# sentiric/sentiric-stt-whisper-service

Hardware: NVIDIA B200
Metric: audio-sec/sec (RTFx) (higher is better)
Workload: dtype bf16 (f32 accumulate)

## Files before the change

include/sw_whisper.h:

```cpp
#ifndef SW_WHISPER_H
#define SW_WHISPER_H

#include <stddef.h>
#include <stdint.h>

#ifdef __cplusplus
extern "C" {
#endif

#define SW_API __attribute__((visibility("default")))

typedef struct sw_ctx sw_ctx;
typedef struct sw_result sw_result;

SW_API const char* sw_last_error(void);
SW_API const char* sw_version(void);
SW_API int sw_device_count(void);

typedef void (*sw_log_callback)(int level, const char* text, void* user);
SW_API void sw_log_set(sw_log_callback cb, void* user);

typedef struct sw_ctx_params {
  int device;
  int max_batch;
// ... 56 lines not shown
                         int n_samples, sw_result** out);
SW_API int sw_full_batch_pcm16(sw_ctx* ctx, const sw_full_params* params,
                               const int16_t* const* pcm16, const int* n_samples, int n,
                               sw_result** out);
SW_API int sw_full_batch_f32(sw_ctx* ctx, const sw_full_params* params, const float* const* pcm,
                             const int* n_samples, int n, sw_result** out);
SW_API int sw_full_batch_pcm16_lang(sw_ctx* ctx, const sw_full_params* params, const int16_t* const* pcm16,
                                    const int* n_samples, int n, const char* const* languages, sw_result** out);
SW_API int sw_full_batch_f32_lang(sw_ctx* ctx, const sw_full_params* params, const float* const* pcm,
                                  const int* n_samples, int n, const char* const* languages, sw_result** out);
SW_API void* sw_host_alloc(size_t bytes);
SW_API void sw_host_free(void* p);

typedef struct sw_token_data {
  int32_t id, tid;
  float p, plog, pt, ptsum;
  int64_t t0, t1, t_dtw;
  float vlen;
} sw_token_data;
SW_API int sw_result_n_segments(const sw_result* r);
SW_API const char* sw_result_segment_text(const sw_result* r, int i);
SW_API int64_t sw_result_segment_t0(const sw_result* r, int i);
SW_API int64_t sw_result_segment_t1(const sw_result* r, int i);
SW_API int sw_result_segment_speaker_turn_next(const sw_result* r, int i);
SW_API int sw_result_n_tokens(const sw_result* r, int i);
SW_API sw_token_data sw_result_token_data(const sw_result* r, int i, int j);
SW_API int sw_result_lang_id(const sw_result* r);
SW_API int sw_result_n_decode_steps(const sw_result* r);
SW_API int sw_result_n_windows(const sw_result* r);
SW_API void sw_result_free(sw_result* r);

typedef struct sw_stats {
  double ms_mel, ms_encode, ms_decode;
  long n_windows, n_steps, n_launches;
  double decode_bytes;
  double decoder_weight_bytes;
  double h2d_bytes, d2h_bytes;
  double ms_xattn;
  long n_xattn;
  double xattn_bytes;
  long n_lanes;
} sw_stats;
SW_API void sw_ctx_set_kernel_timing(sw_ctx* ctx, int on);
SW_API int sw_ctx_get_stats(sw_ctx* ctx, sw_stats* out, int reset);

typedef struct sw_prosody_opts {
  float lpf_alpha, gender_threshold, min_pitch, max_pitch;
} sw_prosody_opts;
enum { SW_EMOTION_NEUTRAL = 0, SW_EMOTION_EXCITED = 1, SW_EMOTION_SAD = 2, SW_EMOTION_ANGRY = 3 };
typedef struct sw_prosody {
  char gender;
  int emotion;
  float arousal, valence, pitch_mean, pitch_std, energy_mean, energy_std, spectral_centroid,
      zero_crossing_rate;
  float speaker_vec[8];
} sw_prosody;
SW_API sw_prosody_opts sw_prosody_default_opts(void);
SW_API int sw_prosody_segments_f32(sw_ctx* ctx, const float* pcm, int64_t n_samples, int sample_rate,
                                   const int64_t* seg_begin, const int64_t* seg_end, int n_segs,
                                   const sw_prosody_opts* opts, sw_prosody* out);
SW_API int sw_prosody_segments_pcm16(sw_ctx* ctx, const int16_t* pcm, int64_t n_samples, int sample_rate,
                                     const int64_t* seg_begin, const int64_t* seg_end, int n_segs,
                                     const sw_prosody_opts* opts, sw_prosody* out);

SW_API int64_t sw_resample_out_len(int64_t n_in, int sr_in, int sr_out);
SW_API int sw_resample_f32(sw_ctx* ctx, const float* in, int64_t n_in, int sr_in, int sr_out, float* out);

SW_API int sw_mel_pcm16(sw_ctx* ctx, const int16_t* pcm, int n_samples, float* out, int* n_len);
SW_API int sw_mel_f32(sw_ctx* ctx, const float* pcm, int n_samples, float* out, int* n_len);
SW_API int sw_encode(sw_ctx* ctx, const float* mel, int n_windows, float* out);
SW_API int sw_decode_logits(sw_ctx* ctx, const int32_t* tokens, int n_windows, int n_tok,
                            float* logits);

SW_API int sw_dev_gemm_bf16(const void* dA, const void* dB, void* dC, const float* d_bias,
                            const float* d_residual, int M, int N, int K, int lda, int ldb, int ldc,
                            int flags, int block_n, void* stream);

SW_API int sw_dev_skinny_gemm(const void* dX, const void* dW, int R, int N, int K, const float* d_bias,
                              int gelu, void* d_out, float* d_partial, int split, void* stream);
SW_API int sw_dev_skinny_split(int N, int K);
SW_API int sw_dev_skinny_gemm_k(int kernel, const void* dX, const void* dW, int R, int N, int K, const float* d_bias,
                                int gelu, void* d_out, float* d_partial, int split, void* stream);
SW_API int sw_dev_skinny_split_k(int kernel, int N, int K);
SW_API int sw_dev_layer_norm(float* d_x, int rows, int d, const float* g, const float* b,
                             void* d_out_bf16, const float* d_partial, int n_split, const float* d_bias,
                             void* stream);
SW_API int sw_dev_occupy(int n_ctas, int smem_bytes, float ms, size_t stream_bytes);

#ifdef __cplusplus
}
#endif
#endif
```

sentiric-stt-whisper-service_b200/csrc/attn_enc_tc.cu:

```cuda
#include <stdlib.h>

#include "common.cuh"
#include "gemm.cuh"
#include "kernels.cuh"

namespace sw {
namespace {

constexpr int TQ = 128, TK = 128, DH = 64;
constexpr int TILE_BYTES = 128 * 64 * 2;
constexpr int SM_Q = 0, SM_K = TILE_BYTES, SM_V = 3 * TILE_BYTES;
constexpr int SM_BARS = 5 * TILE_BYTES;
constexpr int SM_XCH = SM_BARS + 128;
constexpr int ATT_SMEM = SM_XCH + 512;
constexpr int ATT_THREADS = 320;
constexpr int TMEM_COLS = 256, TM_P = 128, TM_O = 192;
#ifndef SW_ATT_POLY
#define SW_ATT_POLY 0
#endif
constexpr bool ATT_POLY = SW_ATT_POLY != 0;

__device__ __forceinline__ uint64_t make_umma_desc_mn_sw128(uint32_t smem_addr) {
  uint64_t d = 0;
  d |= static_cast<uint64_t>((smem_addr >> 4) & 0x3FFF);
  d |= static_cast<uint64_t>(1) << 16;
  d |= static_cast<uint64_t>(64) << 32;
  d |= static_cast<uint64_t>(1) << 46;
  d |= static_cast<uint64_t>(2) << 61;
  return d;
}

__device__ __forceinline__ float fast_exp2(float x) {
  float y;
  asm("ex2.approx.ftz.f32 %0, %1;" : "=f"(y) : "f"(x));
  return y;
}

__device__ __forceinline__ float exp2_fma(float x) {
  x = fmaxf(x, -125.f);
  const float t = x + 12582912.f;
  const float f = x - (t - 12582912.f);
  float p = fmaf(f, 0.05550411f, 0.24022651f);
  p = fmaf(p, f, 0.69314718f);
  p = fmaf(p, f, 1.0f);
  return __int_as_float(__float_as_int(p) + (__float_as_int(t) << 23));
}

template <bool LAGGED>
__global__ void __launch_bounds__(ATT_THREADS, 2)
encoder_attention_tc_kernel(const __grid_constant__ CUtensorMap map_qkv, bf16* __restrict__ out, int T, int d,
                            long long* __restrict__ trace) {
  extern __shared__ __align__(1024) uint8_t smem[];
  uint64_t* bars = reinterpret_cast<uint64_t*>(smem + SM_BARS);
  uint64_t* q_full = bars;
  uint64_t* k_full = bars + 1;
  uint64_t* v_full = bars + 3;
  uint64_t* kv_empty = bars + 5;
  uint64_t* s_full = bars + 7;
  uint64_t* p_ready = bars + 8;
  uint64_t* o_full = bars + 9;
  uint64_t* o_free = bars + 10;
  uint32_t* tmem_slot = reinterpret_cast<uint32_t*>(bars + 11);

  const int qt = blockIdx.x, h = blockIdx.y, w = blockIdx.z;
  const int warp = __shfl_sync(0xffffffffu, threadIdx.x >> 5, 0), lane = threadIdx.x & 31;
  const int q0 = qt * TQ;
  const int n_tiles = (T + TK - 1) / TK;
  const bool tr = trace && blockIdx.x == 5 && blockIdx.y == 7 && blockIdx.z == (gridDim.z >> 1);
#define ATT_TRACE(role, tile, ev)                                                        \
  do {                                                                                   \
    if (tr) trace[((role) * 16 + (tile)) * 8 + (ev)] = clock64();                        \
  } while (0)
  const int row_base = w * T;

  if (threadIdx.x == 0) {
    if (smem_u32(smem) & 1023) {
      printf("encoder_attention_tc: shared memory base not 1024-byte aligned\n");
      __trap();
    }
    tma_prefetch_desc(&map_qkv);
    mbar_init(q_full, 1);
    for (int s = 0; s < 2; ++s) {
      mbar_init(&k_full[s], 1);
      mbar_init(&v_full[s], 1);
      mbar_init(&kv_empty[s], 1);
    }
    mbar_init(s_full, 1);
    mbar_init(p_ready, 8);
    mbar_init(o_full, 1);
    mbar_init(o_free, 8);
    fence_mbar_init();
  }
  if (warp == 1) {
    tmem_alloc(tmem_slot, TMEM_COLS);
    tmem_relinquish();
  }
  tc_fence_before();
  __syncthreads();
  tc_fence_after();
  const uint32_t tmem = *tmem_slot;

  if (warp == 0) {
    if (elect_one_sync()) {
      mbar_arrive_expect_tx(q_full, TILE_BYTES);
      tma_load_2d(smem + SM_Q, &map_qkv, q_full, h * DH, row_base + q0);
      for (int j = 0; j < n_tiles; ++j) {
        const int s = j & 1;
        const uint32_t ph = (j >> 1) & 1;
        mbar_wait(&kv_empty[s], ph ^ 1);
        mbar_arrive_expect_tx(&k_full[s], TILE_BYTES);
        tma_load_2d(smem + SM_K + s * TILE_BYTES, &map_qkv, &k_full[s], d + h * DH, row_base + j * TK);
        mbar_arrive_expect_tx(&v_full[s], TILE_BYTES);
        tma_load_2d(smem + SM_V + s * TILE_BYTES, &map_qkv, &v_full[s], 2 * d + h * DH, row_base + j * TK);
      }
    }
  } else if (warp == 1) {
    if (elect_one_sync()) {
      constexpr uint32_t idesc_s = make_idesc_bf16(128, 128);
      constexpr uint32_t idesc_o = make_idesc_bf16(128, 64) | (1u << 16);
      const uint32_t sq = smem_u32(smem + SM_Q);
      mbar_wait(q_full, 0);
      auto issue_s = [&](int j) {
        const int s = j & 1;
        mbar_wait(&k_full[s], (j >> 1) & 1);
        tc_fence_after();
        const uint64_t adesc = make_umma_desc_sw128(sq);
        const uint64_t bdesc = make_umma_desc_sw128(smem_u32(smem + SM_K + s * TILE_BYTES));
#pragma unroll
        for (int k = 0; k < DH / 16; ++k) umma_bf16(tmem, adesc + 2 * k, bdesc + 2 * k, idesc_s, k != 0);
        umma_commit(s_full);
      };
      issue_s(0);
      for (int j = 0; j < n_tiles; ++j) {
        const int s = j & 1;
        const uint32_t ph = (j >> 1) & 1;
        const uint32_t sv = smem_u32(smem + SM_V + s * TILE_BYTES);
        ATT_TRACE(1, j, 0);
        mbar_wait(p_ready, j & 1);
        tc_fence_after();
        ATT_TRACE(1, j, 1);
        if (j + 1 < n_tiles) issue_s(j + 1);
        ATT_TRACE(1, j, 2);
        mbar_wait(o_free, j & 1);
        tc_fence_after();
        mbar_wait(&v_full[s], ph);
        tc_fence_after();
#pragma unroll
        for (int k = 0; k < TK / 16; ++k) {
          const uint64_t bdesc = make_umma_desc_mn_sw128(sv + k * 2048);
          umma_bf16_ts(tmem + TM_O, tmem + TM_P + k * 8, bdesc, idesc_o, k != 0);
        }
        umma_commit(o_full);
        umma_commit(&kv_empty[s]);
        ATT_TRACE(1, j, 3);
      }
    }
  } else {
    const int qd = warp & 3;
    const int half = (warp - 2) >> 2;
    const int row = qd * 32 + lane;
    const uint32_t lane_addr = static_cast<uint32_t>(qd * 32) << 16;
    const float sc = 0.125f * 1.4426950408889634f;
    float m = -INFINITY, l = 0.f;
    float acc[DH / 2];
#pragma unroll
    for (int i = 0; i < DH / 2; ++i) acc[i] = 0.f;
    uint16_t* xch = reinterpret_cast<uint16_t*>(smem + SM_XCH);
    float alpha_prev = 1.f;
    auto fold_o = [&](int j, float a) {
      mbar_wait(o_full, j & 1);
      tc_fence_after();
      uint32_t r[32];
      tmem_ld_32x32b_x32(tmem + lane_addr + TM_O + half * 32, r);
      tmem_ld_wait(r);
#pragma unroll
      for (int i = 0; i < 32; ++i) acc[i] = acc[i] * a + __uint_as_float(r[i]);
      tc_fence_before();
    };
    const uint32_t s_addr = tmem + lane_addr + half * 64;
    const uint32_t p_addr = tmem + lane_addr + TM_P + half * 32;
    float shift_prev = 0.f;
    for (int j = 0; j < n_tiles; ++j) {
      const int valid = min(TK, T - j * TK);
      mbar_wait(s_full, j & 1);
      tc_fence_after();
      if (warp == 2 && lane == 0) ATT_TRACE(0, j, 0);
      auto exchange_max = [&](float mx) {
        const uint32_t u = __float_as_uint(mx);
        uint32_t t = u & 0xffff0000u;
        if (t != u && !(u >> 31)) t += 0x10000u;
        mx = __uint_as_float(t);
        xch[half * 128 + row] = static_cast<uint16_t>(t >> 16);
        asm volatile("bar.sync 1, 256;" ::: "memory");
        return fmaxf(mx, __uint_as_float(static_cast<uint32_t>(xch[(half ^ 1) * 128 + row]) << 16));
      };
      float lsum = 0.f, mx = -INFINITY;
      auto sweep = [&](float shift, bool want_p) {
        lsum = 0.f;
        mx = -INFINITY;
#pragma unroll
        for (int cc = 0; cc < 2; ++cc) {
          const int c = half * 2 + cc;
          uint32_t r[32];
          tmem_ld_32x32b_x32(s_addr + cc * 32, r);
          tmem_ld_wait(r);
          const bool full = c * 32 + 32 <= valid;
          if (full) {
#pragma unroll
            for (int i = 0; i < 32; ++i) mx = fmaxf(mx, __uint_as_float(r[i]));
          } else {
#pragma unroll
            for (int i = 0; i < 32; ++i)
              if (c * 32 + i < valid) mx = fmaxf(mx, __uint_as_float(r[i]));
          }
          if (!want_p) continue;
          uint32_t pk[16];
          if (full) {
#pragma unroll
            for (int i = 0; i < 16; ++i) {
              const float p0 = fast_exp2(__uint_as_float(r[2 * i]) * sc - shift);
              const float x1 = __uint_as_float(r[2 * i + 1]) * sc - shift;
              const float p1 = (ATT_POLY && i % 3 != 2) ? exp2_fma(x1) : fast_exp2(x1);
              lsum += p0 + p1;
              pk[i] = pack_bf16x2(p0, p1);
            }
          } else {
#pragma unroll
            for (int i = 0; i < 16; ++i) {
              float p0 = fast_exp2(__uint_as_float(r[2 * i]) * sc - shift);
              float p1 = fast_exp2(__uint_as_float(r[2 * i + 1]) * sc - shift);
              if (c * 32 + 2 * i >= valid) p0 = 0.f;
              if (c * 32 + 2 * i + 1 >= valid) p1 = 0.f;
              lsum += p0 + p1;
              pk[i] = pack_bf16x2(p0, p1);
            }
          }
          if (cc == 0 && j > 0) {
            mbar_wait(o_full, (j - 1) & 1);
            tc_fence_after();
          }
          tmem_st_32x32b_x16(p_addr + cc * 16, pk);
        }
      };
      float shift;
      if (!LAGGED || j == 0) {
        sweep(0.f, false);
        if (warp == 2 && lane == 0) ATT_TRACE(0, j, 1);
        mx = exchange_max(mx);
        if (warp == 2 && lane == 0) ATT_TRACE(0, j, 2);
        m = fmaxf(m, mx * sc);
        shift = m;
        sweep(shift, true);
      } else {
        shift = m;
        sweep(shift, true);
        if (warp == 2 && lane == 0) ATT_TRACE(0, j, 1);
        mx = exchange_max(mx);
        if (warp == 2 && lane == 0) ATT_TRACE(0, j, 2);
        m = fmaxf(m, mx * sc);
        if (__any_sync(0xffffffffu, m - shift > 60.f)) {
          shift = m;
          sweep(shift, true);
        }
      }
      const float alpha = j == 0 ? 1.f : fast_exp2(shift_prev - shift);
      shift_prev = shift;
      l = l * alpha + lsum;
      if (warp == 2 && lane == 0) ATT_TRACE(0, j, 3);
      tmem_st_wait();
      tc_fence_before();
      __syncwarp();
      if (lane == 0) mbar_arrive(p_ready);
      if (warp == 2 && lane == 0) ATT_TRACE(0, j, 4);
      if (j > 0) fold_o(j - 1, alpha_prev);
      __syncwarp();
      if (lane == 0) mbar_arrive(o_free);
      if (warp == 2 && lane == 0) ATT_TRACE(0, j, 5);
      alpha_prev = alpha;
    }
    fold_o(n_tiles - 1, alpha_prev);
    float* lx = reinterpret_cast<float*>(smem + SM_K);
    asm volatile("bar.sync 1, 256;" ::: "memory");
    lx[half * 128 + row] = l;
    asm volatile("bar.sync 1, 256;" ::: "memory");
    l += lx[(half ^ 1) * 128 + row];
    if (q0 + row < T) {
      const float inv = 1.0f / l;
      bf16* op = out + (int64_t)(row_base + q0 + row) * d + h * DH + half * 32;
#pragma unroll
      for (int i = 0; i < 4; ++i) {
        uint4 o;
        o.x = pack_bf16x2(acc[8 * i] * inv, acc[8 * i + 1] * inv);
        o.y = pack_bf16x2(acc[8 * i + 2] * inv, acc[8 * i + 3] * inv);
        o.z = pack_bf16x2(acc[8 * i + 4] * inv, acc[8 * i + 5] * inv);
        o.w = pack_bf16x2(acc[8 * i + 6] * inv, acc[8 * i + 7] * inv);
        reinterpret_cast<uint4*>(op)[i] = o;
      }
    }
  }

  tc_fence_before();
  __syncthreads();
  if (warp == 1) {
    tc_fence_after();
    tmem_dealloc(tmem, TMEM_COLS);
  }
}

}

int encoder_attention_tc(const bf16* qkv, bf16* out, int n_win, int T, int d, int n_head, cudaStream_t stream) {
  if (n_win <= 0) return 0;
  SW_CHECK(d == n_head * DH, "encoder_attention: head dim must be 64 (d=%d heads=%d)", d, n_head);
  static SmemOptIn opt_in;
  static SmemOptIn opt_in2;
  SW_CUDA_CHECK(opt_in.ensure(encoder_attention_tc_kernel<true>, ATT_SMEM));
  SW_CUDA_CHECK(opt_in2.ensure(encoder_attention_tc_kernel<false>, ATT_SMEM));
  static const bool lagged = getenv("SW_ATT_LAGGED") && atoi(getenv("SW_ATT_LAGGED")) == 1;
  CUtensorMap map;
  if (make_tma_map_2d_bf16(&map, qkv, 3 * (int64_t)d, (int64_t)n_win * T, 3 * (int64_t)d, 64, 128)) return -1;
  dim3 grid((T + TQ - 1) / TQ, n_head, n_win);
  static int trace_left = getenv("SW_ATTN_TRACE") ? 1 : 0;
  long long* d_trace = nullptr;
  if (trace_left > 0 && n_win >= 8) {
    cudaMalloc(&d_trace, 2 * 16 * 8 * sizeof(long long));
    cudaMemset(d_trace, 0, 2 * 16 * 8 * sizeof(long long));
  }
  if (lagged) encoder_attention_tc_kernel<true><<<grid, ATT_THREADS, ATT_SMEM, stream>>>(map, out, T, d, d_trace);
  else encoder_attention_tc_kernel<false><<<grid, ATT_THREADS, ATT_SMEM, stream>>>(map, out, T, d, d_trace);
  if (d_trace) {
    trace_left = 0;
    long long h[2 * 16 * 8];
    cudaStreamSynchronize(stream);
    cudaMemcpy(h, d_trace, sizeof(h), cudaMemcpyDeviceToHost);
    cudaFree(d_trace);
    const long long t00 = h[0];
    for (int j = 0; j < 12; ++j) {
      const long long* a = h + j * 8;
      const long long* b = h + (16 + j) * 8;
      fprintf(stderr, "[attn trace] tile %2d softmax: S seen %7lld | pass1 %5lld | bar %5lld | pass2 %5lld | fence+arrive %5lld | fold %5lld || "
                      "mma: wait P from %7lld, seen %7lld, PV issued +%4lld, S(j+1) issued +%4lld\n",
              j, a[0] - t00, a[1] - a[0], a[2] - a[1], a[3] - a[2], a[4] - a[3], a[5] - a[4], b[0] - t00, b[1] - t00,
              b[2] - b[1], b[3] - b[2]);
    }
  }
  SW_CUDA_CHECK(cudaGetLastError());
  return 0;
}

}
```

sentiric-stt-whisper-service_b200/csrc/dev_hooks.cu:

```cuda
#include "../../include/sw_whisper.h"
#include "common.cuh"
#include "gemm.cuh"
#include "kernels.cuh"

namespace {
__global__ void __launch_bounds__(512, 1) occupy_kernel(unsigned long long ns, const uint4* __restrict__ buf, size_t n_vec,
                                                       float* sink) {
  extern __shared__ uint8_t occ_smem[];
  float r[96];
#pragma unroll
  for (int i = 0; i < 96; ++i) r[i] = (float)(threadIdx.x + i);
  unsigned long long t0, t;
  asm volatile("mov.u64 %0, %%globaltimer;" : "=l"(t0));
  size_t idx = (size_t)blockIdx.x * blockDim.x + threadIdx.x;
  const size_t stride = (size_t)gridDim.x * blockDim.x;
  uint4 acc = make_uint4(0, 0, 0, 0);
  do {
    if (buf) {
#pragma unroll
      for (int u = 0; u < 8; ++u) {
        const uint4 v = __ldcs(buf + (idx + u * stride) % n_vec);
        acc.x ^= v.x; acc.y ^= v.y; acc.z ^= v.z; acc.w ^= v.w;
      }
      idx += 8 * stride;
// ... 12 lines not shown
extern "C" {

int sw_dev_occupy(int n_ctas, int smem_bytes, float ms, size_t stream_bytes) {
  static cudaStream_t st = nullptr;
  static uint4* buf = nullptr;
  static size_t buf_bytes = 0;
  static float* sink = nullptr;
  if (!st) {
    if (cudaStreamCreateWithFlags(&st, cudaStreamNonBlocking) != cudaSuccess) return -1;
    if (cudaMalloc(&sink, 16) != cudaSuccess) return -1;
  }
  if (n_ctas <= 0) return cudaStreamSynchronize(st) == cudaSuccess ? 0 : -1;
  if (stream_bytes > buf_bytes) {
    if (buf) cudaFree(buf);
    if (cudaMalloc(&buf, stream_bytes) != cudaSuccess) return -1;
    cudaMemsetAsync(buf, 1, stream_bytes, st);
    buf_bytes = stream_bytes;
  }
  if (cudaFuncSetAttribute(occupy_kernel, cudaFuncAttributeMaxDynamicSharedMemorySize, smem_bytes) != cudaSuccess) return -1;
  occupy_kernel<<<n_ctas, 512, smem_bytes, st>>>((unsigned long long)(ms * 1e6), stream_bytes ? buf : nullptr,
                                                  stream_bytes / 16, sink);
  return cudaGetLastError() == cudaSuccess ? 0 : -1;
}

int sw_device_count(void) {
  int n = 0;
  if (cudaGetDeviceCount(&n) != cudaSuccess) {
    cudaGetLastError();
    return 0;
  }
  int ok = 0;
  for (int i = 0; i < n; ++i) {
    int major = 0;
    cudaDeviceGetAttribute(&major, cudaDevAttrComputeCapabilityMajor, i);
    if (major == 10) ++ok;
  }
  return ok;
}

int sw_dev_gemm_bf16(const void* dA, const void* dB, void* dC, const float* d_bias,
                     const float* d_residual, int M, int N, int K, int lda, int ldb, int ldc,
                     int flags, int block_n, void* stream) {
  sw::GemmArgs a;
  a.A = static_cast<const __nv_bfloat16*>(dA);
  a.B = static_cast<const __nv_bfloat16*>(dB);
  a.C = dC;
  a.lda = lda;
  a.ldb = ldb;
  a.ldc = ldc;
  a.bias = d_bias;
  a.residual = d_residual;
  a.ldr = ldc;
  a.M = M;
  a.N = N;
  a.K = K;
  a.flags = flags;
  a.block_n = block_n;
  return sw::gemm_bf16_tn(a, static_cast<cudaStream_t>(stream));
}

int sw_dev_skinny_gemm(const void* dX, const void* dW, int R, int N, int K, const float* d_bias, int gelu,
                       void* d_out, float* d_partial, int split, void* stream) {
  if (split <= 0) split = sw::skinny_split_for(N, K);
  return sw::skinny_gemm(static_cast<const sw::bf16*>(dX), K, static_cast<const sw::bf16*>(dW), R, N, K, d_bias,
                         gelu, static_cast<sw::bf16*>(d_out), N, d_partial, split, static_cast<cudaStream_t>(stream));
}
int sw_dev_skinny_split(int N, int K) { return sw::skinny_split_for(N, K); }
int sw_dev_skinny_gemm_k(int kernel, const void* dX, const void* dW, int R, int N, int K, const float* d_bias, int gelu,
                         void* d_out, float* d_partial, int split, void* stream) {
  const sw::bf16* X = static_cast<const sw::bf16*>(dX);
  const sw::bf16* W = static_cast<const sw::bf16*>(dW);
  cudaStream_t st = static_cast<cudaStream_t>(stream);
  if (kernel == 2) {
    if (split <= 0) split = sw::skinny_tc_split_for(N, K);
    return sw::skinny_gemm_tc(X, K, W, R, N, K, d_bias, gelu, static_cast<sw::bf16*>(d_out), N, d_partial, split, st);
  }
  if (split <= 0) split = kernel == 1 ? sw::skinny_mma_split_for(N, K) : sw::skinny_split_for(N, K);
  return sw::skinny_gemm(X, K, W, R, N, K, d_bias, gelu, static_cast<sw::bf16*>(d_out), N, d_partial, split, st,
                         kernel == 1 ? -1 : 0);
}
int sw_dev_skinny_split_k(int kernel, int N, int K) {
  return kernel == 2 ? sw::skinny_tc_split_for(N, K) : kernel == 1 ? sw::skinny_mma_split_for(N, K) : sw::skinny_split_for(N, K);
}
int sw_dev_layer_norm(float* d_x, int rows, int d, const float* g, const float* b, void* d_out_bf16,
                      const float* d_partial, int n_split, const float* d_bias, void* stream) {
  return sw::layer_norm(d_x, rows, d, g, b, static_cast<sw::bf16*>(d_out_bf16), nullptr, d_partial, n_split,
                        (int64_t)rows * d, d_bias, static_cast<cudaStream_t>(stream));
}
}
```

sentiric-stt-whisper-service_b200/sw_binding.py:

```python
import ctypes as C
import os

import numpy as np

HERE = os.path.dirname(os.path.abspath(__file__))
LIB_PATH = os.environ.get("SW_LIB_PATH") or os.path.join(HERE, "libsw_whisper.so")


class CtxParams(C.Structure):
    _fields_ = [("device", C.c_int), ("max_batch", C.c_int), ("max_beams", C.c_int),
                ("flash_attn", C.c_int), ("n_lanes", C.c_int), ("reserved", C.c_int * 11)]


class ModelInfo(C.Structure):
    _fields_ = [(n, C.c_int) for n in (
        "n_vocab", "n_audio_ctx", "n_audio_state", "n_audio_head", "n_audio_layer", "n_text_ctx",
        "n_text_state", "n_text_head", "n_text_layer", "n_mels", "ftype", "is_multilingual",
        "token_eot", "token_sot", "token_translate", "token_transcribe", "token_solm", "token_prev",
        "token_nosp", "token_not", "token_beg")]


ABORT_CB = C.CFUNCTYPE(C.c_int, C.c_void_p)


class FullParams(C.Structure):
    _fields_ = [
        ("strategy", C.c_int), ("beam_size", C.c_int), ("best_of", C.c_int),
        ("temperature", C.c_float), ("temperature_inc", C.c_float), ("entropy_thold", C.c_float),
        ("logprob_thold", C.c_float), ("no_speech_thold", C.c_float),
        ("translate", C.c_int), ("tdrz_enable", C.c_int), ("suppress_nst", C.c_int),
        ("suppress_blank", C.c_int), ("token_timestamps", C.c_int), ("no_timestamps", C.c_int),
        ("single_segment", C.c_int), ("no_context", C.c_int),
        ("max_initial_ts", C.c_float), ("length_penalty", C.c_float),
        ("language", C.c_char_p), ("initial_prompt", C.c_char_p),
        ("prompt_tokens", C.POINTER(C.c_int32)), ("prompt_n_tokens", C.c_int),
        ("abort_callback", ABORT_CB), ("abort_callback_user_data", C.c_void_p),
        ("n_threads", C.c_int), ("reserved", C.c_int * 8)]


class TokenData(C.Structure):
    _fields_ = [("id", C.c_int32), ("tid", C.c_int32), ("p", C.c_float), ("plog", C.c_float),
                ("pt", C.c_float), ("ptsum", C.c_float), ("t0", C.c_int64), ("t1", C.c_int64),
                ("t_dtw", C.c_int64), ("vlen", C.c_float)]


class Stats(C.Structure):
    _fields_ = [("ms_mel", C.c_double), ("ms_encode", C.c_double), ("ms_decode", C.c_double),
                ("n_windows", C.c_long), ("n_steps", C.c_long), ("n_launches", C.c_long),
                ("decode_bytes", C.c_double), ("decoder_weight_bytes", C.c_double),
                ("h2d_bytes", C.c_double), ("d2h_bytes", C.c_double), ("ms_xattn", C.c_double),
                ("n_xattn", C.c_long), ("xattn_bytes", C.c_double), ("n_lanes", C.c_long)]


class ProsodyOpts(C.Structure):
    _fields_ = [("lpf_alpha", C.c_float), ("gender_threshold", C.c_float), ("min_pitch", C.c_float),
                ("max_pitch", C.c_float)]


class Prosody(C.Structure):
    _fields_ = [("gender", C.c_char), ("emotion", C.c_int), ("arousal", C.c_float), ("valence", C.c_float),
                ("pitch_mean", C.c_float), ("pitch_std", C.c_float), ("energy_mean", C.c_float),
                ("energy_std", C.c_float), ("spectral_centroid", C.c_float), ("zero_crossing_rate", C.c_float),
                ("speaker_vec", C.c_float * 8)]


EMOTIONS = ["neutral", "excited", "sad", "angry"]
PROSODY_FLOATS = ["arousal", "valence", "pitch_mean", "pitch_std", "energy_mean", "energy_std",
                  "spectral_centroid", "zero_crossing_rate"]

EXPORTS = [
    "sw_last_error", "sw_version", "sw_device_count", "sw_log_set", "sw_ctx_default_params",
    "sw_ctx_create", "sw_ctx_destroy", "sw_ctx_model_info", "sw_token_to_str", "sw_token_eot",
    "sw_lang_id", "sw_full_default_params", "sw_full", "sw_full_pcm16", "sw_full_batch_pcm16",
    "sw_full_batch_f32", "sw_full_batch_pcm16_lang", "sw_full_batch_f32_lang", "sw_host_alloc", "sw_host_free", "sw_result_n_segments",
    "sw_result_segment_text", "sw_result_segment_t0", "sw_result_segment_t1",
    "sw_result_segment_speaker_turn_next", "sw_result_n_tokens", "sw_result_token_data",
    "sw_result_lang_id", "sw_result_n_decode_steps", "sw_result_n_windows", "sw_result_free",
    "sw_ctx_get_stats", "sw_ctx_set_kernel_timing", "sw_mel_pcm16", "sw_mel_f32", "sw_encode", "sw_decode_logits",
    "sw_prosody_default_opts", "sw_prosody_segments_f32", "sw_prosody_segments_pcm16",
    "sw_resample_out_len", "sw_resample_f32",
    "sw_dev_gemm_bf16", "sw_dev_skinny_gemm", "sw_dev_skinny_split", "sw_dev_layer_norm", "sw_dev_occupy",
    "sw_dev_skinny_gemm_k", "sw_dev_skinny_split_k"]

_lib = None


def lib():
    global _lib
    if _lib is not None:
        return _lib
    if not os.path.exists(LIB_PATH):
        raise RuntimeError("libsw_whisper.so is not built (run __graft_entry__.build()); "
                           "there is no CPU fallback")
    L = C.CDLL(LIB_PATH)
    vp, ci, fp = C.c_void_p, C.c_int, C.POINTER(C.c_float)
    L.sw_last_error.restype = C.c_char_p
    L.sw_version.restype = C.c_char_p
    L.sw_ctx_default_params.restype = CtxParams
    L.sw_ctx_create.restype = vp
    L.sw_ctx_create.argtypes = [C.c_char_p, C.POINTER(CtxParams)]
    L.sw_ctx_destroy.argtypes = [vp]
    L.sw_ctx_model_info.argtypes = [vp, C.POINTER(ModelInfo)]
    L.sw_token_to_str.restype = C.c_char_p
    L.sw_token_to_str.argtypes = [vp, ci]
    L.sw_token_eot.argtypes = [vp]
    L.sw_lang_id.argtypes = [C.c_char_p]
    L.sw_full_default_params.restype = FullParams
    L.sw_full_default_params.argtypes = [ci]
    L.sw_full.argtypes = [vp, C.POINTER(FullParams), fp, ci, C.POINTER(vp)]
    L.sw_full_pcm16.argtypes = [vp, C.POINTER(FullParams), C.POINTER(C.c_int16), ci, C.POINTER(vp)]
    L.sw_full_batch_pcm16.argtypes = [vp, C.POINTER(FullParams), C.POINTER(C.POINTER(C.c_int16)),
                                      C.POINTER(ci), ci, C.POINTER(vp)]
    L.sw_full_batch_f32.argtypes = [vp, C.POINTER(FullParams), C.POINTER(fp), C.POINTER(ci), ci,
                                    C.POINTER(vp)]
    L.sw_full_batch_pcm16_lang.argtypes = [vp, C.POINTER(FullParams), C.POINTER(C.POINTER(C.c_int16)),
                                           C.POINTER(ci), ci, C.POINTER(C.c_char_p), C.POINTER(vp)]
    L.sw_full_batch_f32_lang.argtypes = [vp, C.POINTER(FullParams), C.POINTER(fp), C.POINTER(ci), ci,
                                         C.POINTER(C.c_char_p), C.POINTER(vp)]
    L.sw_host_alloc.restype = vp
    L.sw_host_alloc.argtypes = [C.c_size_t]
    L.sw_host_free.argtypes = [vp]
    L.sw_result_n_segments.argtypes = [vp]
    L.sw_result_segment_text.restype = C.c_char_p
    L.sw_result_segment_text.argtypes = [vp, ci]
    L.sw_result_segment_t0.restype = C.c_int64
    L.sw_result_segment_t0.argtypes = [vp, ci]
    L.sw_result_segment_t1.restype = C.c_int64
    L.sw_result_segment_t1.argtypes = [vp, ci]
    L.sw_result_segment_speaker_turn_next.argtypes = [vp, ci]
    L.sw_result_n_tokens.argtypes = [vp, ci]
    L.sw_result_token_data.restype = TokenData
    L.sw_result_token_data.argtypes = [vp, ci, ci]
    for n in ("lang_id", "n_decode_steps", "n_windows"):
        getattr(L, "sw_result_" + n).argtypes = [vp]
    L.sw_result_free.argtypes = [vp]
    L.sw_ctx_get_stats.argtypes = [vp, C.POINTER(Stats), ci]
    L.sw_ctx_set_kernel_timing.argtypes = [vp, ci]
    L.sw_mel_pcm16.argtypes = [vp, C.POINTER(C.c_int16), ci, fp, C.POINTER(ci)]
    L.sw_mel_f32.argtypes = [vp, fp, ci, fp, C.POINTER(ci)]
    L.sw_encode.argtypes = [vp, fp, ci, fp]
    L.sw_decode_logits.argtypes = [vp, C.POINTER(C.c_int32), ci, ci, fp]
    _lib = L
    return L


def last_error():
    return lib().sw_last_error().decode(errors="replace")


def _fp(a):
    return a.ctypes.data_as(C.POINTER(C.c_float))


def _tok(t):
    return dict(id=t.id, tid=t.tid, p=t.p, plog=t.plog, pt=t.pt, ptsum=t.ptsum, t0=t.t0, t1=t.t1,
                vlen=t.vlen)


class Engine:
    def __init__(self, model_path, device=0, max_batch=64, max_beams=5, n_lanes=0):
        self.L = lib()
        p = self.L.sw_ctx_default_params()
        p.device, p.max_batch, p.max_beams, p.n_lanes = device, max_batch, max_beams, n_lanes
        self.h = self.L.sw_ctx_create(model_path.encode(), C.byref(p))
        if not self.h:
# ... 163 lines not shown
```

Baseline: 3888.

## Make encoder tcgen05 attention persistent with two Q tiles and TMEM-resident output

Rewrites the Blackwell encoder attention kernel into a persistent grid that loops over work items. Each CTA handles up to two query tiles per item and keeps a three-stage K/V TMA ring plus a double-buffered Q. The output accumulator now stays in TMEM and is rescaled lazily, only when the running max grows past a threshold, instead of being folded into registers every tile. It also uses packed f32x2 FMA/add, drops the tracing and lagged/poly variants, and adds a dev hook for testing. This is meant to cut per-tile softmax work and launch/tail overhead, but it raises smem/TMEM use to one CTA per SM and adds synchronisation complexity.

```diff
diff --git a/include/sw_whisper.h b/include/sw_whisper.h
--- a/include/sw_whisper.h
+++ b/include/sw_whisper.h
@@ -162,6 +162,8 @@
 SW_API int sw_dev_skinny_gemm_k(int kernel, const void* dX, const void* dW, int R, int N, int K, const float* d_bias,
                                 int gelu, void* d_out, float* d_partial, int split, void* stream);
 SW_API int sw_dev_skinny_split_k(int kernel, int N, int K);
+SW_API int sw_dev_encoder_attention(int kernel, const void* d_qkv, void* d_out, int n_win, int T, int d, int n_head,
+                                    void* stream);
 SW_API int sw_dev_layer_norm(float* d_x, int rows, int d, const float* g, const float* b,
                              void* d_out_bf16, const float* d_partial, int n_split, const float* d_bias,
                              void* stream);
diff --git a/sentiric-stt-whisper-service_b200/csrc/attn_enc_tc.cu b/sentiric-stt-whisper-service_b200/csrc/attn_enc_tc.cu
--- a/sentiric-stt-whisper-service_b200/csrc/attn_enc_tc.cu
+++ b/sentiric-stt-whisper-service_b200/csrc/attn_enc_tc.cu
@@ -1,5 +1,3 @@
-#include <stdlib.h>
-
 #include "common.cuh"
 #include "gemm.cuh"
 #include "kernels.cuh"
@@ -9,16 +7,14 @@
 
 constexpr int TQ = 128, TK = 128, DH = 64;
 constexpr int TILE_BYTES = 128 * 64 * 2;
-constexpr int SM_Q = 0, SM_K = TILE_BYTES, SM_V = 3 * TILE_BYTES;
-constexpr int SM_BARS = 5 * TILE_BYTES;
-constexpr int SM_XCH = SM_BARS + 128;
-constexpr int ATT_SMEM = SM_XCH + 512;
+constexpr int NST = 3;
+constexpr int SM_Q = 0;
+constexpr int SM_KV = 4 * TILE_BYTES;
+constexpr int SM_BARS = SM_KV + NST * 2 * TILE_BYTES;
+constexpr int ATT_SMEM = SM_BARS + 256;
 constexpr int ATT_THREADS = 320;
-constexpr int TMEM_COLS = 256, TM_P = 128, TM_O = 192;
-#ifndef SW_ATT_POLY
-#define SW_ATT_POLY 0
-#endif
-constexpr bool ATT_POLY = SW_ATT_POLY != 0;
+constexpr int TMEM_COLS = 512, TM_TILE = 256, TM_P = 128, TM_O = 192;
+constexpr float RESCALE_LOG2 = 8.f;
 
 __device__ __forceinline__ uint64_t make_umma_desc_mn_sw128(uint32_t smem_addr) {
   uint64_t d = 0;
@@ -35,43 +31,73 @@
   asm("ex2.approx.ftz.f32 %0, %1;" : "=f"(y) : "f"(x));
   return y;
 }
-
-__device__ __forceinline__ float exp2_fma(float x) {
-  x = fmaxf(x, -125.f);
-  const float t = x + 12582912.f;
-  const float f = x - (t - 12582912.f);
-  float p = fmaf(f, 0.05550411f, 0.24022651f);
-  p = fmaf(p, f, 0.69314718f);
-  p = fmaf(p, f, 1.0f);
-  return __int_as_float(__float_as_int(p) + (__float_as_int(t) << 23));
-}
-
-template <bool LAGGED>
-__global__ void __launch_bounds__(ATT_THREADS, 2)
+__device__ __forceinline__ void ffma2(float& dx, float& dy, float ax, float ay, float bx, float by, float cx, float cy) {
+  asm("{\n\t.reg .b64 ra, rb, rc, rd;\n\tmov.b64 ra, {%2, %3};\n\tmov.b64 rb, {%4, %5};\n\tmov.b64 rc, {%6, %7};\n\t"
+      "fma.rn.ftz.f32x2 rd, ra, rb, rc;\n\tmov.b64 {%0, %1}, rd;\n\t}"
+      : "=f"(dx), "=f"(dy)
+      : "f"(ax), "f"(ay), "f"(bx), "f"(by), "f"(cx), "f"(cy));
+}
+__device__ __forceinline__ void fadd2(float& dx, float& dy, float ax, float ay, float bx, float by) {
+  asm("{\n\t.reg .b64 ra, rb, rd;\n\tmov.b64 ra, {%2, %3};\n\tmov.b64 rb, {%4, %5};\n\t"
+      "add.rn.ftz.f32x2 rd, ra, rb;\n\tmov.b64 {%0, %1}, rd;\n\t}"
+      : "=f"(dx), "=f"(dy)
+      : "f"(ax), "f"(ay), "f"(bx), "f"(by));
+}
+__device__ __forceinline__ void fmul2(float& dx, float& dy, float ax, float ay, float b) {
+  asm("{\n\t.reg .b64 ra, rb, rd;\n\tmov.b64 ra, {%2, %3};\n\tmov.b64 rb, {%4, %4};\n\t"
+      "mul.rn.ftz.f32x2 rd, ra, rb;\n\tmov.b64 {%0, %1}, rd;\n\t}"
+      : "=f"(dx), "=f"(dy)
+      : "f"(ax), "f"(ay), "f"(b));
+}
+__device__ __forceinline__ float fmax3(float a, float b, float c) {
+  float d;
+  asm("max.f32 %0, %1, %2, %3;" : "=f"(d) : "f"(a), "f"(b), "f"(c));
+  return d;
+}
+
+__device__ __forceinline__ void tmem_ld_32x32b_x16(uint32_t taddr, uint32_t (&r)[16]) {
+  asm volatile(
+      "tcgen05.ld.sync.aligned.32x32b.x16.b32 {%0, %1, %2, %3, %4, %5, %6, %7, %8, %9, %10, %11, %12, %13, %14, %15}, "
+      "[%16];\n\ttcgen05.wait::ld.sync.aligned;"
+      : "=r"(r[0]), "=r"(r[1]), "=r"(r[2]), "=r"(r[3]), "=r"(r[4]), "=r"(r[5]), "=r"(r[6]), "=r"(r[7]), "=r"(r[8]),
+        "=r"(r[9]), "=r"(r[10]), "=r"(r[11]), "=r"(r[12]), "=r"(r[13]), "=r"(r[14]), "=r"(r[15])
+      : "r"(taddr)
+      : "memory");
+}
+
+struct Item {
+  int w, h, qt0, nt;
+};
+__device__ __forceinline__ Item decode_item(int item, int n_head, int tpi, int q_tiles) {
+  const int ipp = (q_tiles + tpi - 1) / tpi;
+  Item it;
+  const int p = item % ipp;
+  const int wh = item / ipp;
+  it.h = wh % n_head;
+  it.w = wh / n_head;
+  it.qt0 = p * tpi;
+  it.nt = min(tpi, q_tiles - it.qt0);
+  return it;
+}
+
+__global__ void __launch_bounds__(ATT_THREADS, 1)
 encoder_attention_tc_kernel(const __grid_constant__ CUtensorMap map_qkv, bf16* __restrict__ out, int T, int d,
-                            long long* __restrict__ trace) {
+                            int n_head, int tpi, int n_items) {
   extern __shared__ __align__(1024) uint8_t smem[];
   uint64_t* bars = reinterpret_cast<uint64_t*>(smem + SM_BARS);
   uint64_t* q_full = bars;
-  uint64_t* k_full = bars + 1;
-  uint64_t* v_full = bars + 3;
-  uint64_t* kv_empty = bars + 5;
-  uint64_t* s_full = bars + 7;
-  uint64_t* p_ready = bars + 8;
-  uint64_t* o_full = bars + 9;
-  uint64_t* o_free = bars + 10;
-  uint32_t* tmem_slot = reinterpret_cast<uint32_t*>(bars + 11);
-
-  const int qt = blockIdx.x, h = blockIdx.y, w = blockIdx.z;
+  uint64_t* q_empty = bars + 2;
+  uint64_t* kv_full = bars + 4;
+  uint64_t* kv_empty = bars + 4 + NST;
+  uint64_t* s_full = bars + 4 + 2 * NST;
+  uint64_t* p_ready = bars + 6 + 2 * NST;
+  uint64_t* o_done = bars + 8 + 2 * NST;
+  uint64_t* s_free = bars + 10 + 2 * NST;
+  uint32_t* tmem_slot = reinterpret_cast<uint32_t*>(bars + 12 + 2 * NST);
+
   const int warp = __shfl_sync(0xffffffffu, threadIdx.x >> 5, 0), lane = threadIdx.x & 31;
-  const int q0 = qt * TQ;
-  const int n_tiles = (T + TK - 1) / TK;
-  const bool tr = trace && blockIdx.x == 5 && blockIdx.y == 7 && blockIdx.z == (gridDim.z >> 1);
-#define ATT_TRACE(role, tile, ev)                                                        \
-  do {                                                                                   \
-    if (tr) trace[((role) * 16 + (tile)) * 8 + (ev)] = clock64();                        \
-  } while (0)
-  const int row_base = w * T;
+  const int q_tiles = (T + TQ - 1) / TQ;
+  const int n_kt = (T + TK - 1) / TK;
 
   if (threadIdx.x == 0) {
     if (smem_u32(smem) & 1023) {
@@ -79,16 +105,18 @@
       __trap();
     }
     tma_prefetch_desc(&map_qkv);
-    mbar_init(q_full, 1);
-    for (int s = 0; s < 2; ++s) {
-      mbar_init(&k_full[s], 1);
-      mbar_init(&v_full[s], 1);
+    for (int i = 0; i < 2; ++i) {
+      mbar_init(&q_full[i], 1);
+      mbar_init(&q_empty[i], 1);
+      mbar_init(&s_full[i], 1);
+      mbar_init(&p_ready[i], 4);
+      mbar_init(&s_free[i], 4);
+      mbar_init(&o_done[i], 1);
+    }
+    for (int s = 0; s < NST; ++s) {
+      mbar_init(&kv_full[s], 1);
       mbar_init(&kv_empty[s], 1);
     }
-    mbar_init(s_full, 1);
-    mbar_init(p_ready, 8);
-    mbar_init(o_full, 1);
-    mbar_init(o_free, 8);
     fence_mbar_init();
   }
   if (warp == 1) {
@@ -102,199 +130,198 @@
 
   if (warp == 0) {
     if (elect_one_sync()) {
-      mbar_arrive_expect_tx(q_full, TILE_BYTES);
-      tma_load_2d(smem + SM_Q, &map_qkv, q_full, h * DH, row_base + q0);
-      for (int j = 0; j < n_tiles; ++j) {
-        const int s = j & 1;
-        const uint32_t ph = (j >> 1) & 1;
-        mbar_wait(&kv_empty[s], ph ^ 1);
-        mbar_arrive_expect_tx(&k_full[s], TILE_BYTES);
-        tma_load_2d(smem + SM_K + s * TILE_BYTES, &map_qkv, &k_full[s], d + h * DH, row_base + j * TK);
-        mbar_arrive_expect_tx(&v_full[s], TILE_BYTES);
-        tma_load_2d(smem + SM_V + s * TILE_BYTES, &map_qkv, &v_full[s], 2 * d + h * DH, row_base + j * TK);
+      int kv = 0, k = 0;
+      for (int item = blockIdx.x; item < n_items; item += gridDim.x, ++k) {
+        const Item it = decode_item(item, n_head, tpi, q_tiles);
+        const int row_base = it.w * T;
+        const int qb = k & 1;
+        mbar_wait(&q_empty[qb], ((k >> 1) & 1) ^ 1);
+        mbar_arrive_expect_tx(&q_full[qb], it.nt * TILE_BYTES);
+        for (int t = 0; t < it.nt; ++t)
+          tma_load_2d(smem + SM_Q + (qb * 2 + t) * TILE_BYTES, &map_qkv, &q_full[qb], it.h * DH,
+                      row_base + (it.qt0 + t) * TQ);
+        for (int j = 0; j < n_kt; ++j, ++kv) {
+          const int s = kv % NST;
+          mbar_wait(&kv_empty[s], ((kv / NST) & 1) ^ 1);
+          uint8_t* st = smem + SM_KV + s * 2 * TILE_BYTES;
+          mbar_arrive_expect_tx(&kv_full[s], 2 * TILE_BYTES);
+          tma_load_2d(st, &map_qkv, &kv_full[s], d + it.h * DH, row_base + j * TK);
+          tma_load_2d(st + TILE_BYTES, &map_qkv, &kv_full[s], 2 * d + it.h * DH, row_base + j * TK);
+        }
       }
     }
   } else if (warp == 1) {
     if (elect_one_sync()) {
       constexpr uint32_t idesc_s = make_idesc_bf16(128, 128);
       constexpr uint32_t idesc_o = make_idesc_bf16(128, 64) | (1u << 16);
-      const uint32_t sq = smem_u32(smem + SM_Q);
-      mbar_wait(q_full, 0);
-      auto issue_s = [&](int j) {
-        const int s = j & 1;
-        mbar_wait(&k_full[s], (j >> 1) & 1);
+      uint32_t pr[2] = {0u, 0u}, sf[2] = {0u, 0u};
+      int kv = 0, k = 0;
+      auto issue_s = [&](int qb, int t, int kvi) {
+        const uint64_t adesc = make_umma_desc_sw128(smem_u32(smem + SM_Q + (qb * 2 + t) * TILE_BYTES));
+        const uint64_t bdesc = make_umma_desc_sw128(smem_u32(smem + SM_KV + (kvi % NST) * 2 * TILE_BYTES));
+#pragma unroll
+        for (int kk = 0; kk < DH / 16; ++kk)
+          umma_bf16(tmem + t * TM_TILE, adesc + 2 * kk, bdesc + 2 * kk, idesc_s, kk != 0);
+        umma_commit(&s_full[t]);
+      };
+      for (int item = blockIdx.x; item < n_items; item += gridDim.x, ++k) {
+        const Item it = decode_item(item, n_head, tpi, q_tiles);
+        const int qb = k & 1;
+        mbar_wait(&q_full[qb], (k >> 1) & 1);
+        mbar_wait(&kv_full[kv % NST], (kv / NST) & 1);
         tc_fence_after();
-        const uint64_t adesc = make_umma_desc_sw128(sq);
-        const uint64_t bdesc = make_umma_desc_sw128(smem_u32(smem + SM_K + s * TILE_BYTES));
-#pragma unroll
-        for (int k = 0; k < DH / 16; ++k) umma_bf16(tmem, adesc + 2 * k, bdesc + 2 * k, idesc_s, k != 0);
-        umma_commit(s_full);
-      };
-      issue_s(0);
-      for (int j = 0; j < n_tiles; ++j) {
-        const int s = j & 1;
-        const uint32_t ph = (j >> 1) & 1;
-        const uint32_t sv = smem_u32(smem + SM_V + s * TILE_BYTES);
-        ATT_TRACE(1, j, 0);
-        mbar_wait(p_ready, j & 1);
+        for (int t = 0; t < it.nt; ++t) issue_s(qb, t, kv);
+        for (int j = 0; j < n_kt; ++j) {
+          const int kvj = kv + j;
+          const uint32_t sv = smem_u32(smem + SM_KV + (kvj % NST) * 2 * TILE_BYTES + TILE_BYTES);
+          if (j + 1 < n_kt) {
+            mbar_wait(&kv_full[(kvj + 1) % NST], ((kvj + 1) / NST) & 1);
+            tc_fence_after();
+          }
+          for (int t = 0; t < it.nt; ++t) {
+            mbar_wait(&s_free[t], sf[t] & 1);
+            ++sf[t];
+            tc_fence_after();
+            if (j + 1 < n_kt) issue_s(qb, t, kvj + 1);
+          }
+          for (int t = 0; t < it.nt; ++t) {
+            mbar_wait(&p_ready[t], pr[t] & 1);
+            ++pr[t];
+            tc_fence_after();
+            const uint32_t tt = tmem + t * TM_TILE;
+#pragma unroll
+            for (int kk = 0; kk < TK / 16; ++kk) {
+              const uint64_t bdesc = make_umma_desc_mn_sw128(sv + kk * 2048);
+              umma_bf16_ts(tt + TM_O, tt + TM_P + kk * 8, bdesc, idesc_o, (j | kk) != 0);
+            }
+            umma_commit(&o_done[t]);
+          }
+          umma_commit(&kv_empty[kvj % NST]);
+        }
+        umma_commit(&q_empty[qb]);
+        kv += n_kt;
+      }
+    }
+  } else {
+    const int t = (warp - 2) >> 2;
+    const int qd = warp & 3;
+    const int row = qd * 32 + lane;
+    const uint32_t tbase = tmem + t * TM_TILE + (static_cast<uint32_t>(qd * 32) << 16);
+    const float sc = 0.125f * 1.4426950408889634f;
+    uint32_t sp = 0, op = 0;
+    for (int item = blockIdx.x; item < n_items; item += gridDim.x) {
+      const Item it = decode_item(item, n_head, tpi, q_tiles);
+      if (t >= it.nt) continue;
+      float m = -INFINITY, l = 0.f;
+      for (int j = 0; j < n_kt; ++j) {
+        mbar_wait(&s_full[t], sp & 1);
+        ++sp;
         tc_fence_after();
-        ATT_TRACE(1, j, 1);
-        if (j + 1 < n_tiles) issue_s(j + 1);
-        ATT_TRACE(1, j, 2);
-        mbar_wait(o_free, j & 1);
-        tc_fence_after();
-        mbar_wait(&v_full[s], ph);
-        tc_fence_after();
-#pragma unroll
-        for (int k = 0; k < TK / 16; ++k) {
-          const uint64_t bdesc = make_umma_desc_mn_sw128(sv + k * 2048);
-          umma_bf16_ts(tmem + TM_O, tmem + TM_P + k * 8, bdesc, idesc_o, k != 0);
-        }
-        umma_commit(o_full);
-        umma_commit(&kv_empty[s]);
-        ATT_TRACE(1, j, 3);
+        uint32_t r[4][32];
+#pragma unroll
+        for (int c = 0; c < 4; ++c) tmem_ld_32x32b_x32(tbase + c * 32, r[c]);
+#pragma unroll
+        for (int c = 0; c < 4; ++c) tmem_ld_wait(r[c]);
+        tc_fence_before();
+        __syncwarp();
+        if (lane == 0) mbar_arrive(&s_free[t]);
+        const int valid = T - j * TK;
+        if (valid < TK) {
+#pragma unroll
+          for (int c = 0; c < 4; ++c)
+#pragma unroll
+            for (int i = 0; i < 32; ++i)
+              if (c * 32 + i >= valid) r[c][i] = __float_as_uint(-INFINITY);
+        }
+        float mx[4];
+#pragma unroll
+        for (int c = 0; c < 4; ++c) {
+          mx[c] = __uint_as_float(r[c][0]);
+#pragma unroll
+          for (int i = 1; i < 31; i += 2) mx[c] = fmax3(mx[c], __uint_as_float(r[c][i]), __uint_as_float(r[c][i + 1]));
+          mx[c] = fmaxf(mx[c], __uint_as_float(r[c][31]));
+        }
+        const float mt = fmaxf(fmax3(mx[0], mx[1], mx[2]), mx[3]) * sc;
+        const bool need = mt > m + RESCALE_LOG2;
+        float alpha = 1.f;
+        if (need) {
+          alpha = fast_exp2(m - mt);
+          m = mt;
+        }
+        bool o_ready = j == 0;
+        if (j > 0 && __any_sync(0xffffffffu, need)) {
+          mbar_wait(&o_done[t], op & 1);
+          ++op;
+          tc_fence_after();
+          o_ready = true;
+#pragma unroll 1
+          for (int c = 0; c < DH; c += 16) {
+            uint32_t o[16];
+            tmem_ld_32x32b_x16(tbase + TM_O + c, o);
+#pragma unroll
+            for (int i = 0; i < 16; i += 2) {
+              float a, b;
+              fmul2(a, b, __uint_as_float(o[i]), __uint_as_float(o[i + 1]), alpha);
+              o[i] = __float_as_uint(a);
+              o[i + 1] = __float_as_uint(b);
+            }
+            tmem_st_32x32b_x16(tbase + TM_O + c, o);
+          }
+        }
+        const float nm = -m;
+        float s0 = 0.f, s1 = 0.f, s2 = 0.f, s3 = 0.f;
+#pragma unroll
+        for (int c = 0; c < 4; ++c) {
+          uint32_t pk[16];
+#pragma unroll
+          for (int i = 0; i < 16; ++i) {
+            float x0, x1;
+            ffma2(x0, x1, __uint_as_float(r[c][2 * i]), __uint_as_float(r[c][2 * i + 1]), sc, sc, nm, nm);
+            x0 = fast_exp2(x0);
+            x1 = fast_exp2(x1);
+            if (i & 1) fadd2(s2, s3, s2, s3, x0, x1);
+            else fadd2(s0, s1, s0, s1, x0, x1);
+            pk[i] = pack_bf16x2(x0, x1);
+          }
+          if (c == 0 && !o_ready) {
+            mbar_wait(&o_done[t], op & 1);
+            ++op;
+            tc_fence_after();
+          }
+          tmem_st_32x32b_x16(tbase + TM_P + c * 16, pk);
+        }
+        fadd2(s0, s1, s0, s1, s2, s3);
+        l = fmaf(l, alpha, s0 + s1);
+        tmem_st_wait();
+        tc_fence_before();
+        __syncwarp();
+        if (lane == 0) mbar_arrive(&p_ready[t]);
       }
-    }
-  } else {
-    const int qd = warp & 3;
-    const int half = (warp - 2) >> 2;
-    const int row = qd * 32 + lane;
-    const uint32_t lane_addr = static_cast<uint32_t>(qd * 32) << 16;
-    const float sc = 0.125f * 1.4426950408889634f;
-    float m = -INFINITY, l = 0.f;
-    float acc[DH / 2];
-#pragma unroll
-    for (int i = 0; i < DH / 2; ++i) acc[i] = 0.f;
-    uint16_t* xch = reinterpret_cast<uint16_t*>(smem + SM_XCH);
-    float alpha_prev = 1.f;
-    auto fold_o = [&](int j, float a) {
-      mbar_wait(o_full, j & 1);
+      mbar_wait(&o_done[t], op & 1);
+      ++op;
       tc_fence_after();
-      uint32_t r[32];
-      tmem_ld_32x32b_x32(tmem + lane_addr + TM_O + half * 32, r);
-      tmem_ld_wait(r);
-#pragma unroll
-      for (int i = 0; i < 32; ++i) acc[i] = acc[i] * a + __uint_as_float(r[i]);
+      uint32_t o[2][32];
+      tmem_ld_32x32b_x32(tbase + TM_O, o[0]);
+      tmem_ld_32x32b_x32(tbase + TM_O + 32, o[1]);
+      tmem_ld_wait(o[0]);
+      tmem_ld_wait(o[1]);
       tc_fence_before();
-    };
-    const uint32_t s_addr = tmem + lane_addr + half * 64;
-    const uint32_t p_addr = tmem + lane_addr + TM_P + half * 32;
-    float shift_prev = 0.f;
-    for (int j = 0; j < n_tiles; ++j) {
-      const int valid = min(TK, T - j * TK);
-      mbar_wait(s_full, j & 1);
-      tc_fence_after();
-      if (warp == 2 && lane == 0) ATT_TRACE(0, j, 0);
-      auto exchange_max = [&](float mx) {
-        const uint32_t u = __float_as_uint(mx);
-        uint32_t t = u & 0xffff0000u;
-        if (t != u && !(u >> 31)) t += 0x10000u;
-        mx = __uint_as_float(t);
-        xch[half * 128 + row] = static_cast<uint16_t>(t >> 16);
-        asm volatile("bar.sync 1, 256;" ::: "memory");
-        return fmaxf(mx, __uint_as_float(static_cast<uint32_t>(xch[(half ^ 1) * 128 + row]) << 16));
-      };
-      float lsum = 0.f, mx = -INFINITY;
-      auto sweep = [&](float shift, bool want_p) {
-        lsum = 0.f;
-        mx = -INFINITY;
-#pragma unroll
-        for (int cc = 0; cc < 2; ++cc) {
-          const int c = half * 2 + cc;
-          uint32_t r[32];
-          tmem_ld_32x32b_x32(s_addr + cc * 32, r);
-          tmem_ld_wait(r);
-          const bool full = c * 32 + 32 <= valid;
-          if (full) {
-#pragma unroll
-            for (int i = 0; i < 32; ++i) mx = fmaxf(mx, __uint_as_float(r[i]));
-          } else {
-#pragma unroll
-            for (int i = 0; i < 32; ++i)
-              if (c * 32 + i < valid) mx = fmaxf(mx, __uint_as_float(r[i]));
-          }
-          if (!want_p) continue;
-          uint32_t pk[16];
-          if (full) {
-#pragma unroll
-            for (int i = 0; i < 16; ++i) {
-              const float p0 = fast_exp2(__uint_as_float(r[2 * i]) * sc - shift);
-              const float x1 = __uint_as_float(r[2 * i + 1]) * sc - shift;
-              const float p1 = (ATT_POLY && i % 3 != 2) ? exp2_fma(x1) : fast_exp2(x1);
-              lsum += p0 + p1;
-              pk[i] = pack_bf16x2(p0, p1);
-            }
-          } else {
-#pragma unroll
-            for (int i = 0; i < 16; ++i) {
-              float p0 = fast_exp2(__uint_as_float(r[2 * i]) * sc - shift);
-              float p1 = fast_exp2(__uint_as_float(r[2 * i + 1]) * sc - shift);
-              if (c * 32 + 2 * i >= valid) p0 = 0.f;
-              if (c * 32 + 2 * i + 1 >= valid) p1 = 0.f;
-              lsum += p0 + p1;
-              pk[i] = pack_bf16x2(p0, p1);
-            }
-          }
-          if (cc == 0 && j > 0) {
-            mbar_wait(o_full, (j - 1) & 1);
-            tc_fence_after();
-          }
-          tmem_st_32x32b_x16(p_addr + cc * 16, pk);
-        }
-      };
-      float shift;
-      if (!LAGGED || j == 0) {
-        sweep(0.f, false);
-        if (warp == 2 && lane == 0) ATT_TRACE(0, j, 1);
-        mx = exchange_max(mx);
-        if (warp == 2 && lane == 0) ATT_TRACE(0, j, 2);
-        m = fmaxf(m, mx * sc);
-        shift = m;
-        sweep(shift, true);
-      } else {
-        shift = m;
-        sweep(shift, true);
-        if (warp == 2 && lane == 0) ATT_TRACE(0, j, 1);
-        mx = exchange_max(mx);
-        if (warp == 2 && lane == 0) ATT_TRACE(0, j, 2);
-        m = fmaxf(m, mx * sc);
-        if (__any_sync(0xffffffffu, m - shift > 60.f)) {
-          shift = m;
-          sweep(shift, true);
-        }
-      }
-      const float alpha = j == 0 ? 1.f : fast_exp2(shift_prev - shift);
-      shift_prev = shift;
-      l = l * alpha + lsum;
-      if (warp == 2 && lane == 0) ATT_TRACE(0, j, 3);
-      tmem_st_wait();
-      tc_fence_before();
-      __syncwarp();
-      if (lane == 0) mbar_arrive(p_ready);
-      if (warp == 2 && lane == 0) ATT_TRACE(0, j, 4);
-      if (j > 0) fold_o(j - 1, alpha_prev);
-      __syncwarp();
-      if (lane == 0) mbar_arrive(o_free);
-      if (warp == 2 && lane == 0) ATT_TRACE(0, j, 5);
-      alpha_prev = alpha;
-    }
-    fold_o(n_tiles - 1, alpha_prev);
-    float* lx = reinterpret_cast<float*>(smem + SM_K);
-    asm volatile("bar.sync 1, 256;" ::: "memory");
-    lx[half * 128 + row] = l;
-    asm volatile("bar.sync 1, 256;" ::: "memory");
-    l += lx[(half ^ 1) * 128 + row];
-    if (q0 + row < T) {
-      const float inv = 1.0f / l;
-      bf16* op = out + (int64_t)(row_base + q0 + row) * d + h * DH + half * 32;
-#pragma unroll
-      for (int i = 0; i < 4; ++i) {
-        uint4 o;
-        o.x = pack_bf16x2(acc[8 * i] * inv, acc[8 * i + 1] * inv);
-        o.y = pack_bf16x2(acc[8 * i + 2] * inv, acc[8 * i + 3] * inv);
-        o.z = pack_bf16x2(acc[8 * i + 4] * inv, acc[8 * i + 5] * inv);
-        o.w = pack_bf16x2(acc[8 * i + 6] * inv, acc[8 * i + 7] * inv);
-        reinterpret_cast<uint4*>(op)[i] = o;
+      const int q = (it.qt0 + t) * TQ + row;
+      if (q < T) {
+        const float inv = 1.0f / l;
+        bf16* dst = out + (int64_t)(it.w * T + q) * d + it.h * DH;
+#pragma unroll
+        for (int c = 0; c < 2; ++c)
+#pragma unroll
+          for (int i = 0; i < 4; ++i) {
+            const uint32_t* v = &o[c][8 * i];
+            uint4 u;
+            u.x = pack_bf16x2(__uint_as_float(v[0]) * inv, __uint_as_float(v[1]) * inv);
+            u.y = pack_bf16x2(__uint_as_float(v[2]) * inv, __uint_as_float(v[3]) * inv);
+            u.z = pack_bf16x2(__uint_as_float(v[4]) * inv, __uint_as_float(v[5]) * inv);
+            u.w = pack_bf16x2(__uint_as_float(v[6]) * inv, __uint_as_float(v[7]) * inv);
+            reinterpret_cast<uint4*>(dst)[c * 4 + i] = u;
+          }
       }
     }
   }
@@ -310,40 +337,20 @@
 }
 
 int encoder_attention_tc(const bf16* qkv, bf16* out, int n_win, int T, int d, int n_head, cudaStream_t stream) {
-  if (n_win <= 0) return 0;
+  if (n_win <= 0 || T <= 0) return 0;
   SW_CHECK(d == n_head * DH, "encoder_attention: head dim must be 64 (d=%d heads=%d)", d, n_head);
   static SmemOptIn opt_in;
-  static SmemOptIn opt_in2;
-  SW_CUDA_CHECK(opt_in.ensure(encoder_attention_tc_kernel<true>, ATT_SMEM));
-  SW_CUDA_CHECK(opt_in2.ensure(encoder_attention_tc_kernel<false>, ATT_SMEM));
-  static const bool lagged = getenv("SW_ATT_LAGGED") && atoi(getenv("SW_ATT_LAGGED")) == 1;
+  SW_CUDA_CHECK(opt_in.ensure(encoder_attention_tc_kernel, ATT_SMEM));
   CUtensorMap map;
   if (make_tma_map_2d_bf16(&map, qkv, 3 * (int64_t)d, (int64_t)n_win * T, 3 * (int64_t)d, 64, 128)) return -1;
-  dim3 grid((T + TQ - 1) / TQ, n_head, n_win);
-  static int trace_left = getenv("SW_ATTN_TRACE") ? 1 : 0;
-  long long* d_trace = nullptr;
-  if (trace_left > 0 && n_win >= 8) {
-    cudaMalloc(&d_trace, 2 * 16 * 8 * sizeof(long long));
-    cudaMemset(d_trace, 0, 2 * 16 * 8 * sizeof(long long));
-  }
-  if (lagged) encoder_attention_tc_kernel<true><<<grid, ATT_THREADS, ATT_SMEM, stream>>>(map, out, T, d, d_trace);
-  else encoder_attention_tc_kernel<false><<<grid, ATT_THREADS, ATT_SMEM, stream>>>(map, out, T, d, d_trace);
-  if (d_trace) {
-    trace_left = 0;
-    long long h[2 * 16 * 8];
-    cudaStreamSynchronize(stream);
-    cudaMemcpy(h, d_trace, sizeof(h), cudaMemcpyDeviceToHost);
-    cudaFree(d_trace);
-    const long long t00 = h[0];
-    for (int j = 0; j < 12; ++j) {
-      const long long* a = h + j * 8;
-      const long long* b = h + (16 + j) * 8;
-      fprintf(stderr, "[attn trace] tile %2d softmax: S seen %7lld | pass1 %5lld | bar %5lld | pass2 %5lld | fence+arrive %5lld | fold %5lld || "
-                      "mma: wait P from %7lld, seen %7lld, PV issued +%4lld, S(j+1) issued +%4lld\n",
-              j, a[0] - t00, a[1] - a[0], a[2] - a[1], a[3] - a[2], a[4] - a[3], a[5] - a[4], b[0] - t00, b[1] - t00,
-              b[2] - b[1], b[3] - b[2]);
-    }
-  }
+  const int sms = device_sm_count();
+  const int q_tiles = (T + TQ - 1) / TQ;
+  const int64_t pairs = (int64_t)n_win * n_head * ((q_tiles + 1) / 2);
+  const int tpi = pairs >= sms ? 2 : 1;
+  const int64_t n_items = (int64_t)n_win * n_head * ((q_tiles + tpi - 1) / tpi);
+  SW_CHECK(n_items < (1ll << 31), "encoder_attention: %lld work items", (long long)n_items);
+  const int grid = (int)(n_items < sms ? n_items : sms);
+  encoder_attention_tc_kernel<<<grid, ATT_THREADS, ATT_SMEM, stream>>>(map, out, T, d, n_head, tpi, (int)n_items);
   SW_CUDA_CHECK(cudaGetLastError());
   return 0;
 }
diff --git a/sentiric-stt-whisper-service_b200/csrc/dev_hooks.cu b/sentiric-stt-whisper-service_b200/csrc/dev_hooks.cu
--- a/sentiric-stt-whisper-service_b200/csrc/dev_hooks.cu
+++ b/sentiric-stt-whisper-service_b200/csrc/dev_hooks.cu
@@ -118,6 +118,14 @@
 int sw_dev_skinny_split_k(int kernel, int N, int K) {
   return kernel == 2 ? sw::skinny_tc_split_for(N, K) : kernel == 1 ? sw::skinny_mma_split_for(N, K) : sw::skinny_split_for(N, K);
 }
+int sw_dev_encoder_attention(int kernel, const void* d_qkv, void* d_out, int n_win, int T, int d, int n_head,
+                             void* stream) {
+  const sw::bf16* qkv = static_cast<const sw::bf16*>(d_qkv);
+  sw::bf16* out = static_cast<sw::bf16*>(d_out);
+  cudaStream_t st = static_cast<cudaStream_t>(stream);
+  return kernel == 1 ? sw::encoder_attention(qkv, out, n_win, T, d, n_head, st)
+                     : sw::encoder_attention_tc(qkv, out, n_win, T, d, n_head, st);
+}
 int sw_dev_layer_norm(float* d_x, int rows, int d, const float* g, const float* b, void* d_out_bf16,
                       const float* d_partial, int n_split, const float* d_bias, void* stream) {
   return sw::layer_norm(d_x, rows, d, g, b, static_cast<sw::bf16*>(d_out_bf16), nullptr, d_partial, n_split,
diff --git a/sentiric-stt-whisper-service_b200/sw_binding.py b/sentiric-stt-whisper-service_b200/sw_binding.py
--- a/sentiric-stt-whisper-service_b200/sw_binding.py
+++ b/sentiric-stt-whisper-service_b200/sw_binding.py
@@ -80,7 +80,7 @@
     "sw_prosody_default_opts", "sw_prosody_segments_f32", "sw_prosody_segments_pcm16",
     "sw_resample_out_len", "sw_resample_f32",
     "sw_dev_gemm_bf16", "sw_dev_skinny_gemm", "sw_dev_skinny_split", "sw_dev_layer_norm", "sw_dev_occupy",
-    "sw_dev_skinny_gemm_k", "sw_dev_skinny_split_k"]
+    "sw_dev_skinny_gemm_k", "sw_dev_skinny_split_k", "sw_dev_encoder_attention"]
 
 _lib = None
 
```

New measurement: 3966, median of 6. 1.02x the previous value.
